# ZhengyiLuo/PULSE

Hardware: NVIDIA H100
Metric: env-steps/sec at 16384 humanoid envs, 1/2/4/8 H100; obs-kernel HBM GB/s (higher is better)
Workload: dtype bf16 GEMM operands, fp32 accumulate / master weights / observations

## Files before the change

### include/pulse_b200.h

```cpp
#ifndef PULSE_B200_H_
#define PULSE_B200_H_

#include <stdint.h>

#ifdef __cplusplus
extern "C" {
#endif

#define PULSE_ABI_VERSION 3

enum pulse_status {
  PULSE_OK = 0,
  PULSE_ERR_ARG = -1,
  PULSE_ERR_CUDA = -2,
  PULSE_ERR_UNSUPPORTED = -3
};

#define PULSE_NUM_BODIES 24
#define PULSE_NUM_DOF 69
#define PULSE_BODY_STATE_W 13
#define PULSE_SELF_OBS 358
#define PULSE_TASK_OBS_V6 576
#define PULSE_IM_OBS (PULSE_SELF_OBS + PULSE_TASK_OBS_V6)
#define PULSE_AMP_OBS 196
// ... 232 lines not shown

typedef struct {
  const float* bias;
  int32_t act;
  int32_t gate_mode;
  const pulse_bf16_t* gate;
  int64_t ldg;
  float alpha;
  pulse_bf16_t* out;
  int64_t ldo;
  pulse_bf16_t* out_t;
  int64_t ldot;
  float* out_f32;
  int64_t ldf;
  int64_t split_stride;
  pulse_bf16_t* preact;
  int64_t ldp;
  float* colsum;
  int32_t accumulate;
  int32_t reserved;
  double* sumsq;
  uint32_t* relu_mask; int64_t ld_rmask;
  const uint32_t* gate_mask; int64_t ld_gmask;
} pulse_gemm_epilogue_t;

#define PULSE_GEMM_A_MN 1u
#define PULSE_GEMM_B_MN 2u

int pulse_gemm_bf16(const void* a, int64_t lda, const void* b, int64_t ldb, int64_t m, int64_t n, int64_t k,
                    const pulse_gemm_epilogue_t* ep, int32_t split_k, uint32_t flags, void* stream);
int pulse_gemm_num_splits(int64_t k, int32_t split_k);
int pulse_gemm_tile_n(int64_t m, int64_t n, int64_t k, int32_t split_k, int32_t sms);
int pulse_gemm_last_tile_n(void);

int pulse_normalize_to_bf16(const float* x, int64_t ldx, int64_t rows, int64_t cols, const float* mean, const float* rstd,
                            pulse_bf16_t* out, int64_t ld_out, pulse_bf16_t* out_t, int64_t ld_t, float pad_one, void* stream);

int pulse_column_moments(const float* x, int64_t ldx, int64_t rows, int64_t cols, double* sums, void* stream);

int pulse_normalize_moments(const float* x, int64_t ldx, int64_t rows, int64_t cols, const float* mean, const float* rstd,
                            pulse_bf16_t* out, int64_t ld_out, double* sums, float pad_one, void* stream);

int pulse_normalize_split(const float* x, int64_t ldx, int64_t rows, int64_t cols, int64_t self_cols, const float* mean, const float* rstd,
                          pulse_bf16_t* p, int64_t ldp, int64_t p_off, pulse_bf16_t* t, int64_t ldt, double* sums, void* stream);

int pulse_rms_merge(double* sums, int64_t n, int32_t size, double* mean, double* var, double* count, float eps,
                    float* mean_f32, float* rstd_f32, void* stream);

int pulse_head1_forward(const pulse_bf16_t* h, int64_t ldh, int64_t rows, int32_t k, const pulse_bf16_t* w, const float* bias, float* out,
                        int64_t ldo, void* stream);

#define PULSE_HEAD1_MAX_CTAS 264
int pulse_head1_backward(const pulse_bf16_t* h, int64_t ldh, int64_t rows, int32_t k, const pulse_bf16_t* dv, int64_t ld_dv,
                         const pulse_bf16_t* w, pulse_bf16_t* dh, int64_t ld_dh, float* dw, float* db, float* dbias_prev, float* partials,
                         void* stream);

int pulse_ordered_sum_add(const float* x, int64_t n, int64_t stride_n, int64_t rows, int64_t cols, int64_t ld, float* out, int64_t ldo,
                          void* stream);

int pulse_gaussian_sample(const float* mu, int64_t ld_mu, const float* eps, const float* logstd, int64_t rows, int32_t num_actions,
                          float* actions, float* neglogp, void* stream);

typedef struct {
  const float* mu; int64_t ld_mu;
  const float* value; int64_t ld_value;
  const float* actions;
// ... 304 lines not shown
```

### pulse_b200/_lib.py

```python
import ctypes as C
import os

_PKG = os.path.dirname(os.path.abspath(__file__))
LIB_PATH = os.path.join(_PKG, "libpulse_b200.so")


class PulseError(RuntimeError):
    pass


c_float_p = C.POINTER(C.c_float)
c_i64_p = C.POINTER(C.c_int64)
c_i32_p = C.POINTER(C.c_int32)
c_u8_p = C.POINTER(C.c_uint8)
c_f64_p = C.POINTER(C.c_double)


class MotionLibDesc(C.Structure):
    _fields_ = [
        ("gts", C.c_void_p), ("grs", C.c_void_p), ("lrs", C.c_void_p), ("gvs", C.c_void_p), ("gavs", C.c_void_p),
        ("dvs", C.c_void_p), ("motion_aa", C.c_void_p), ("lengths", C.c_void_p), ("dt", C.c_void_p),
        ("num_frames", C.c_void_p), ("length_starts", C.c_void_p), ("total_frames", C.c_int64),
        ("num_motions", C.c_int64), ("frame_rec", C.c_void_p), ("aux_rec", C.c_void_p),
    ]
# ... 282 lines not shown
HEAD1_MAX_CTAS = 264
ACT_NONE, ACT_RELU, ACT_SILU = 0, 1, 2
Z_SAMPLE, Z_MEAN, Z_RESIDUAL = 0, 1, 2
STEP_REWARD, STEP_RESET, STEP_OBS, STEP_ALL, STEP_ADVANCE = 1, 2, 4, 7, 8
GETUP_REF, GETUP_FALL, GETUP_RECOVERY = 1, 2, 3

SIGNATURES = {
    "pulse_abi_version": (C.c_int, []),
    "pulse_last_error": (C.c_char_p, []),
    "pulse_launch_count": (C.c_int64, []),
    "pulse_motionlib_create": (C.c_int, [C.POINTER(MotionLibDesc), C.c_void_p, C.POINTER(C.c_void_p)]),
    "pulse_motionlib_destroy": (C.c_int, [C.c_void_p]),
    "pulse_motion_state": (C.c_int, [C.c_void_p, C.POINTER(MotionQuery), C.c_int64, C.c_void_p]),
    "pulse_im_step": (C.c_int, [C.c_void_p, C.POINTER(ImStepArgs), C.c_int64, C.c_void_p]),
    "pulse_reset_ref_state": (C.c_int, [C.c_void_p, C.POINTER(ResetArgs), C.c_int64, C.c_void_p]),
    "pulse_reset_getup": (C.c_int, [C.c_void_p, C.POINTER(GetupResetArgs), C.c_int64, C.c_void_p]),
    "pulse_getup_amp_init": (C.c_int, [C.POINTER(GetupAmpArgs), C.c_int64, C.c_void_p]),
    "pulse_policy_post": (C.c_int, [C.POINTER(PolicyPostArgs), C.c_int64, C.c_void_p]),
    "pulse_value_post": (C.c_int, [C.c_void_p, C.c_int64, C.c_void_p, C.c_void_p, C.c_float, C.c_void_p, C.c_void_p, C.c_int64, C.c_int64, C.c_void_p]),
    "pulse_amp_obs_row": (C.c_int, [C.POINTER(AmpRowArgs), C.c_int64, C.c_void_p]),
    "pulse_bump_counter": (C.c_int, [C.c_void_p, C.c_uint64, C.c_void_p]),
    "pulse_event_create": (C.c_int, [C.POINTER(C.c_void_p)]),
    "pulse_event_destroy": (C.c_int, [C.c_void_p]),
    "pulse_event_record": (C.c_int, [C.c_void_p, C.c_void_p]),
    "pulse_event_elapsed_ms": (C.c_int, [C.c_void_p, C.c_void_p, C.POINTER(C.c_float)]),
    "pulse_amp_obs": (C.c_int, [C.POINTER(AmpObsArgs), C.c_int64, C.c_void_p]),
    "pulse_gae": (C.c_int, [C.POINTER(GaeArgs), C.c_int32, C.c_int64, C.c_void_p]),
    "pulse_normalize_advantages": (C.c_int, [C.c_void_p, C.c_void_p, C.c_int64, C.c_void_p]),
    "pulse_gemm_bf16": (C.c_int, [C.c_void_p, C.c_int64, C.c_void_p, C.c_int64, C.c_int64, C.c_int64, C.c_int64,
                                  C.POINTER(GemmEpilogue), C.c_int32, C.c_uint32, C.c_void_p]),
    "pulse_gemm_num_splits": (C.c_int, [C.c_int64, C.c_int32]),
    "pulse_gemm_tile_n": (C.c_int, [C.c_int64, C.c_int64, C.c_int64, C.c_int32, C.c_int32]),
    "pulse_gemm_last_tile_n": (C.c_int, []),
    "pulse_normalize_to_bf16": (C.c_int, [C.c_void_p, C.c_int64, C.c_int64, C.c_int64, C.c_void_p, C.c_void_p, C.c_void_p, C.c_int64,
                                          C.c_void_p, C.c_int64, C.c_float, C.c_void_p]),
    "pulse_normalize_moments": (C.c_int, [C.c_void_p, C.c_int64, C.c_int64, C.c_int64, C.c_void_p, C.c_void_p, C.c_void_p, C.c_int64,
                                          C.c_void_p, C.c_float, C.c_void_p]),
    "pulse_normalize_split": (C.c_int, [C.c_void_p, C.c_int64, C.c_int64, C.c_int64, C.c_int64, C.c_void_p, C.c_void_p, C.c_void_p, C.c_int64,
                                        C.c_int64, C.c_void_p, C.c_int64, C.c_void_p, C.c_void_p]),
    "pulse_head1_forward": (C.c_int, [C.c_void_p, C.c_int64, C.c_int64, C.c_int32, C.c_void_p, C.c_void_p, C.c_void_p, C.c_int64, C.c_void_p]),
    "pulse_head1_backward": (C.c_int, [C.c_void_p, C.c_int64, C.c_int64, C.c_int32, C.c_void_p, C.c_int64, C.c_void_p, C.c_void_p, C.c_int64,
                                       C.c_void_p, C.c_void_p, C.c_void_p, C.c_void_p, C.c_void_p]),
    "pulse_ordered_sum_add": (C.c_int, [C.c_void_p, C.c_int64, C.c_int64, C.c_int64, C.c_int64, C.c_int64, C.c_void_p, C.c_int64, C.c_void_p]),
    "pulse_column_moments": (C.c_int, [C.c_void_p, C.c_int64, C.c_int64, C.c_int64, C.c_void_p, C.c_void_p]),
    "pulse_rms_merge": (C.c_int, [C.c_void_p, C.c_int64, C.c_int32, C.c_void_p, C.c_void_p, C.c_void_p, C.c_float, C.c_void_p, C.c_void_p,
                                  C.c_void_p]),
    "pulse_gaussian_sample": (C.c_int, [C.c_void_p, C.c_int64, C.c_void_p, C.c_void_p, C.c_int64, C.c_int32, C.c_void_p, C.c_void_p,
                                        C.c_void_p]),
    "pulse_ppo_loss": (C.c_int, [C.POINTER(PpoLossArgs), C.c_int64, C.c_void_p]),
    "pulse_disc_loss": (C.c_int, [C.c_void_p, C.c_int64, C.c_int64, C.c_int64, C.c_float, C.c_void_p, C.c_int64, C.c_void_p, C.c_void_p]),
    "pulse_relu_mask_scale": (C.c_int, [C.c_void_p, C.c_int64, C.c_int64, C.c_int64, C.c_void_p, C.c_void_p, C.c_int64, C.c_void_p]),
    "pulse_weight_reg": (C.c_int, [C.POINTER(WeightReg), C.c_void_p]),
    "pulse_axpy": (C.c_int, [C.c_float, C.c_void_p, C.c_void_p, C.c_int64, C.c_void_p]),
    "pulse_column_sum_bf16": (C.c_int, [C.c_void_p, C.c_int64, C.c_int64, C.c_int64, C.c_void_p, C.c_void_p]),
    "pulse_reduce_slabs": (C.c_int, [C.c_void_p, C.c_int64, C.c_int32, C.c_int64, C.c_void_p, C.c_void_p]),
    "pulse_sum_squares": (C.c_int, [C.c_void_p, C.c_int64, C.c_void_p, C.c_void_p]),
    "pulse_adam_step": (C.c_int, [C.c_void_p, C.c_void_p, C.c_void_p, C.c_void_p, C.c_int64, C.c_void_p, C.c_float, C.c_float,
                                  C.c_float, C.c_float, C.c_float, C.c_void_p, C.c_void_p, C.c_uint32, C.c_void_p, C.c_void_p]),
    "pulse_peer_reduce_adam": (C.c_int, [C.POINTER(PeerAdamArgs), C.c_void_p]),
    "pulse_refresh_weight_bf16": (C.c_int, [C.c_void_p, C.c_int64, C.c_int64, C.c_void_p, C.c_int64, C.c_void_p, C.c_int64, C.c_void_p]),
    "pulse_normalize_cols": (C.c_int, [C.c_void_p, C.c_int64, C.c_int64, C.c_int64, C.c_void_p, C.c_void_p, C.c_float, C.c_void_p, C.c_int64,
                                       C.c_int64, C.c_void_p]),
    "pulse_copy_cols_bf16": (C.c_int, [C.c_void_p, C.c_int64, C.c_int64, C.c_int64, C.c_void_p, C.c_int64, C.c_void_p, C.c_int64, C.c_void_p]),
    "pulse_vae_reparam": (C.c_int, [C.c_void_p, C.c_int64, C.c_void_p, C.c_int64, C.c_int64, C.c_int32, C.c_int32, C.c_int32, C.c_float,
                                    C.c_float, C.c_void_p, C.c_int64, C.c_void_p, C.c_int64, C.c_void_p]),
    "pulse_vae_reparam_philox": (C.c_int, [C.c_void_p, C.c_int64, C.c_int64, C.c_int32, C.c_int32, C.c_float, C.c_float, C.c_uint64,
# ... 84 lines not shown
```

### pulse_b200/csrc/gemm_kernel.inc

```

template <bool A_MN, bool B_MN, int MODE, int S, int BN>
__global__ void __launch_bounds__(kThreads, 1) gemm_bf16_kernel(const __grid_constant__ CUtensorMap map_a,
                                                                const __grid_constant__ CUtensorMap map_b,
                                                                const __grid_constant__ CUtensorMap map_c,
                                                                const __grid_constant__ CUtensorMap map_p,
                                                                const pulse_gemm_epilogue_t ep, int M, int N, int K,
                                                                int kb_per_split, int splits, int tma_out) {
  constexpr bool kFwd = MODE == kModeGeneric || MODE == kModeFwd;
  constexpr bool kDgrad = MODE == kModeGeneric || MODE == kModeDgrad || MODE == kModeDgradVec;
  constexpr bool kGateVec = MODE == kModeGeneric || MODE == kModeDgradVec;
  constexpr bool kAccum = MODE == kModeGeneric || MODE == kModeWgrad;
  constexpr bool kBf16Out = MODE != kModeWgrad;
  constexpr bool kRegEpi = MODE == kModeFwd || MODE == kModeDgrad;
  constexpr bool kWide = BN == kWideBN;
  constexpr bool kStaged = S == kStages && !kWide;
  static_assert(kStaged || kRegEpi, "deep-ring and wide instantiations run the register-resident epilogue only");
  static_assert(!kWide || (S == kStages && !A_MN), "wide tiles: 4-stage ring, K-major A");
  constexpr bool kPreRoom = sizeof(GemmSmem<S, BN>::epi[0]) >= 32768;
  extern __shared__ unsigned char gsm_raw[];
  GemmSmem<S, BN>& sm = *reinterpret_cast<GemmSmem<S, BN>*>((reinterpret_cast<uintptr_t>(gsm_raw) + 1023) & ~static_cast<uintptr_t>(1023));
  const int warp = threadIdx.x >> 5, lane = threadIdx.x & 31;
  const int work0 = static_cast<int>(blockIdx.x);
  const int work_stride = static_cast<int>(gridDim.x);
  const int tiles_n = (N + BN - 1) / BN, tiles_m = (M + BM - 1) / BM;
  const int tiles = tiles_m * tiles_n;
  const int total = tiles * splits;
  const int num_kb_total = (K + BK - 1) / BK;
  if (threadIdx.x == 0) PULSE_TRACE_START();

  if (threadIdx.x == 0) {
#pragma unroll
    for (int s = 0; s < S; ++s) {
      g_mbar_init(&sm.full[s], 1);
      g_mbar_init(&sm.empty[s], kConsumerWarps);
    }
    asm volatile("fence.mbarrier_init.release.cluster;\n" ::: "memory");
    asm volatile("prefetch.tensormap [%0];\n" ::"l"(&map_a) : "memory");
    asm volatile("prefetch.tensormap [%0];\n" ::"l"(&map_b) : "memory");
  }
  __syncthreads();
  if (threadIdx.x == 0) PULSE_TRACE(1);
  asm volatile("griddepcontrol.launch_dependents;\n" ::: "memory");

  if (warp < 4) {
    if constexpr (kWide) asm volatile("setmaxnreg.dec.sync.aligned.u32 %0;\n" ::"n"(kWideProducerRegs));
    if (warp == 0 && lane == 0) {
      asm volatile("griddepcontrol.wait;\n" ::: "memory");
      PULSE_TRACE(2);
      int it = 0, lw = 0;
      for (int w = work0; w < total; w += work_stride, ++lw) {
        const int split = w / tiles, t = w - split * tiles;
        const int m0 = (t / tiles_n) * BM, n0 = (t % tiles_n) * BN;
        const int kb0 = split * kb_per_split;
        const int num_kb = min(kb_per_split, num_kb_total - kb0);
        long long empty_clk = 0;
        (void)empty_clk;
        if (lw < 3) PULSE_TRACE_SET(25 + lw, num_kb);
        for (int kb = 0; kb < num_kb; ++kb, ++it) {
          const int s = it % S;
          PULSE_RING_WAIT(&sm.empty[s], ((it / S) & 1) ^ 1, empty_clk);
          g_mbar_expect_tx(&sm.full[s], kStageBytesA + BN * BK * 2);
          const int kk = (kb0 + kb) * BK;
          if (A_MN) {
            tma_load_2d(sm.a[s], &map_a, m0, kk, &sm.full[s]);
            tma_load_2d(sm.a[s] + 8192, &map_a, m0 + 64, kk, &sm.full[s]);
          } else {
            tma_load_2d(sm.a[s], &map_a, kk, m0, &sm.full[s]);
          }
          if (B_MN) {
#pragma unroll
            for (int i = 0; i < BN / 64; ++i) tma_load_2d(sm.b[s] + 8192 * i, &map_b, n0 + 64 * i, kk, &sm.full[s]);
          } else {
            tma_load_2d(sm.b[s], &map_b, kk, n0, &sm.full[s]);
          }
        }
        if (lw < 3) PULSE_TRACE_SET(28 + lw, empty_clk);
      }
    }
  } else {
    if constexpr (kWide) asm volatile("setmaxnreg.inc.sync.aligned.u32 %0;\n" ::"n"(kWideConsumerRegs));
    const int wg = (warp >> 2) - 1;
    const int ew = warp - 4;
    const int quarter = wg * 2 + (warp & 1);
    const int chalf = (warp >> 1) & 1;
    float* red_stage = nullptr;
    float* acc_s = nullptr;
    if constexpr (kStaged) {
      red_stage = sm.red[ew];
      acc_s = sm.epi[wg];
    }
    asm volatile("griddepcontrol.wait;\n" ::: "memory");
    int it = 0, lw = 0;
    for (int w = work0; w < total; w += work_stride, ++lw) {
      const int split = w / tiles, t = w - split * tiles;
      const int m0 = (t / tiles_n) * BM, n0 = (t % tiles_n) * BN;
      const int kb0 = split * kb_per_split;
      const int num_kb = min(kb_per_split, num_kb_total - kb0);
      const bool reg_epi = !kStaged || (kRegEpi && tma_out);
      const int r0 = (warp & 3) * 16 + (lane >> 2);
      const int row = m0 + quarter * 32 + lane;
      const bool row_ok = row < M;
      const bool gate_fast = kStaged && (MODE == kModeGeneric || MODE == kModeDgrad) && ep.gate != nullptr && ep.gate_mask == nullptr && ep.gate_mode == PULSE_ACT_RELU && (ep.ldg & 7) == 0 && n0 + chalf * kCols + kCols <= N;
      unsigned gmask[BN / 16] = {};
      const bool gate_bits = kDgrad && ep.gate_mask != nullptr;
      if (gate_bits && reg_epi) {
#pragma unroll
        for (int c = 0; c < BN / 32; ++c) {
#pragma unroll
          for (int h = 0; h < 2; ++h) {
            const int r = m0 + wg * 64 + r0 + 8 * h;
            if (r < M && n0 + c * 32 < N) gmask[2 * c + h] = __ldg(ep.gate_mask + static_cast<long long>((n0 >> 5) + c) * ep.ld_gmask + r);
          }
        }
      } else if (gate_bits && row_ok) {
#pragma unroll
        for (int cc = 0; cc < kChunks; ++cc) {
          const int col = n0 + (chalf * kChunks + cc) * 32;
          if (col < N) gmask[cc] = __ldg(ep.gate_mask + static_cast<long long>(col >> 5) * ep.ld_gmask + row);
        }
      }
      if (gate_fast && row_ok) {
        const uint4* g = reinterpret_cast<const uint4*>(reinterpret_cast<const __nv_bfloat16*>(ep.gate) + static_cast<long long>(row) * ep.ldg +
                                                        n0 + chalf * kCols);
        uint4 u[kChunks * 4];
#pragma unroll
        for (int i = 0; i < kChunks * 4; ++i) u[i] = __ldg(g + i);
#pragma unroll
        for (int i = 0; i < kChunks * 4; ++i) {
// ... 22 lines not shown
          const int t = (warp & 3) * 32 + lane;
          sm.bias[wg][t] = n0 + t < N ? __ldg(ep.bias + n0 + t) : 0.0f;
        }
      } else if (kFwd && ep.bias != nullptr) {
#pragma unroll
        for (int cc = 0; cc < kChunks; ++cc) {
          const int col = n0 + (chalf * kChunks + cc) * 32 + lane;
          if (col < N) bias_l[cc] = __ldg(ep.bias + col);
        }
      }

      float d[BN / 2];
#pragma unroll
      for (int i = 0; i < BN / 2; ++i) d[i] = 0.0f;
      acc_fence(d);
      int prev_s = -1;
      long long full_clk = 0;
      (void)full_clk;
      for (int kb = 0; kb < num_kb; ++kb, ++it) {
        const int s = it % S;
        PULSE_RING_WAIT(&sm.full[s], (it / S) & 1, full_clk);
        if (it == 0 && ew == 0 && lane == 0) PULSE_TRACE(3);
        wgmma_fence();
        const unsigned a_addr = s_u32(sm.a[s]) + static_cast<unsigned>(wg) * 8192u, b_addr = s_u32(sm.b[s]);
#pragma unroll
        for (int k = 0; k < BK / MMA_K; ++k) {
          const unsigned long long da = A_MN ? gmma_desc(a_addr + k * 2048, 8192) : gmma_desc(a_addr + k * 32, 16);
          const unsigned long long db = B_MN ? gmma_desc(b_addr + k * 2048, 8192) : gmma_desc(b_addr + k * 32, 16);
          if constexpr (kWide) wgmma_m64n256<A_MN ? 1 : 0, B_MN ? 1 : 0>(d, da, db, (kb | k) != 0 ? 1u : 0u);
          else wgmma_m64n128<A_MN ? 1 : 0, B_MN ? 1 : 0>(d, da, db, (kb | k) != 0 ? 1u : 0u);
        }
        wgmma_commit();
        wgmma_wait<1>();
        if (prev_s >= 0 && lane == 0) g_mbar_arrive(&sm.empty[prev_s]);
        prev_s = s;
      }
      wgmma_wait<0>();
      acc_fence(d);
      if (lane == 0) g_mbar_arrive(&sm.empty[prev_s]);
      if (ew == 0 && lane == 0 && lw < 3) {
        PULSE_TRACE(4 + lw);
        PULSE_TRACE_SET(22 + lw, full_clk);
      }

      if (kRegEpi && (warp & 3) == 0 && lane == 0) asm volatile("cp.async.bulk.wait_group.read 0;\n" ::: "memory");
      wg_sync(wg);
      float sq = 0.0f;

      if (reg_epi) {
        const int q = lane & 3;
        if (ep.alpha != 1.0f) {
#pragma unroll
          for (int i = 0; i < BN / 2; ++i) d[i] *= ep.alpha;
        }
        if (kFwd && ep.bias != nullptr) {
#pragma unroll
          for (int j = 0; j < BN / 8; ++j) {
            float2 b;
            if constexpr (kWide) {
              const int c = n0 + 8 * j + 2 * q;
              b = make_float2(c < N ? __ldg(ep.bias + c) : 0.0f, c + 1 < N ? __ldg(ep.bias + c + 1) : 0.0f);
            } else {
              b = *reinterpret_cast<const float2*>(sm.bias[wg] + 2 * q + 8 * j);
            }
            d[4 * j] += b.x; d[4 * j + 1] += b.y; d[4 * j + 2] += b.x; d[4 * j + 3] += b.y;
          }
        }
        if (kFwd && ep.relu_mask != nullptr) {
#pragma unroll
          for (int hf = 0; hf < BN / 128; ++hf) {
            unsigned wd[4][2];
#pragma unroll
// ... 275 lines not shown
              for (int i = 0; i < 32; ++i)
                if (col0 + i < N) p[i] = v[i];
            }
          }
          if (kBf16Out && ep.out != nullptr) {
            if (full && (ep.ldo & 7) == 0) {
              store_block_bf16(reinterpret_cast<uint4*>(red_stage), v,
                               reinterpret_cast<__nv_bfloat16*>(ep.out) + static_cast<long long>(m0 + quarter * 32) * ep.ldo + col0, ep.ldo,
                               M - (m0 + quarter * 32), lane);
            } else if (row_ok) {
              __nv_bfloat16* p = reinterpret_cast<__nv_bfloat16*>(ep.out) + static_cast<long long>(row) * ep.ldo + col0;
  #pragma unroll
              for (int i = 0; i < 32; ++i)
                if (col0 + i < N) p[i] = __float2bfloat16(v[i]);
            }
          }
          if (kFwd && ep.out_t != nullptr && row_ok) {
  #pragma unroll
            for (int i = 0; i < 32; ++i)
              if (col0 + i < N)
                reinterpret_cast<__nv_bfloat16*>(ep.out_t)[static_cast<long long>(col0 + i) * ep.ldot + row] = __float2bfloat16(v[i]);
          }
        }
        if (MODE == kModeWgrad && tma_out) {
          if (lane == 0) asm volatile("cp.async.bulk.wait_group.read 0;\n" ::: "memory");
          __syncwarp();
        }
        if (kDgrad && ep.sumsq != nullptr) add_sumsq(ep.sumsq, sq);
        if (ew == 0 && lane == 0 && lw < 3) PULSE_TRACE(17 + 2 * lw);
      }
    }
  }
  if ((MODE == kModeWgrad || kRegEpi) && warp >= 4 && lane == 0) asm volatile("cp.async.bulk.wait_group 0;\n" ::: "memory");
  if (threadIdx.x == 0) PULSE_TRACE(10);
}
```

### pulse_b200/csrc/gemm_wgmma.cu

```cuda
#include <cuda.h>
#include <stdlib.h>
#include <string.h>
#include <cuda_bf16.h>

#include "pulse_common.cuh"

namespace pulse {
namespace {

#ifndef PULSE_GEMM_VARIANT
#define PULSE_GEMM_VARIANT 0
#endif
constexpr int BM = 128, BK = 64, MMA_K = 16;
constexpr int kNarrowBN = 128, kWideBN = 256;
constexpr int kConsumerWarps = 8;
constexpr int kThreads = 128 + 32 * kConsumerWarps;
constexpr int kCols = 64;
constexpr int kChunks = kCols / 32;
constexpr int kStages = 4;
constexpr int kTmaOutF32 = 2;
constexpr unsigned kStageBytesA = BM * BK * 2;
constexpr int kWideProducerRegs = 40, kWideConsumerRegs = 232;

template <int S, int BN>
// ... 31 lines not shown
              "GEMM shared-memory layout exceeds the per-block opt-in limit");

__device__ __forceinline__ unsigned s_u32(const void* p) { return static_cast<unsigned>(__cvta_generic_to_shared(p)); }
__device__ __forceinline__ void g_mbar_init(unsigned long long* bar, unsigned count) {
  asm volatile("mbarrier.init.shared::cta.b64 [%0], %1;\n" ::"r"(s_u32(bar)), "r"(count));
}
__device__ __forceinline__ void g_mbar_expect_tx(unsigned long long* bar, unsigned bytes) {
  asm volatile("mbarrier.arrive.expect_tx.shared::cta.b64 _, [%0], %1;\n" ::"r"(s_u32(bar)), "r"(bytes) : "memory");
}
__device__ __forceinline__ void g_mbar_arrive(unsigned long long* bar) {
  asm volatile("mbarrier.arrive.shared::cta.b64 _, [%0];\n" ::"r"(s_u32(bar)) : "memory");
}
__device__ __forceinline__ bool g_mbar_try(unsigned long long* bar, unsigned parity) {
  unsigned ok;
  asm volatile(
      "{\n\t.reg .pred p;\n\t"
      "mbarrier.try_wait.parity.shared::cta.b64 p, [%1], %2;\n\t"
      "selp.u32 %0, 1, 0, p;\n\t}\n"
      : "=r"(ok)
      : "r"(s_u32(bar)), "r"(parity)
      : "memory");
  return ok != 0;
}
__device__ __forceinline__ void g_mbar_wait(unsigned long long* bar, unsigned parity) {
  for (int spin = 0; spin < (1 << 26); ++spin)
    if (g_mbar_try(bar, parity)) return;
  __trap();
}
__device__ __forceinline__ void tma_load_2d(void* smem_dst, const CUtensorMap* map, int c0, int c1, unsigned long long* bar) {
  asm volatile("cp.async.bulk.tensor.2d.shared::cluster.global.mbarrier::complete_tx::bytes [%0], [%1, {%3, %4}], [%2];\n" ::"r"(
                   s_u32(smem_dst)),
               "l"(map), "r"(s_u32(bar)), "r"(c0), "r"(c1)
               : "memory");
}
__device__ __forceinline__ void tma_store_2d(const CUtensorMap* map, unsigned smem_src, int c0, int c1) {
  asm volatile("cp.async.bulk.tensor.2d.global.shared::cta.bulk_group [%0, {%2, %3}], [%1];\n" ::"l"(map), "r"(smem_src), "r"(c0), "r"(c1)
               : "memory");
}
__device__ __forceinline__ void tma_store_3d(const CUtensorMap* map, unsigned smem_src, int c0, int c1, int c2) {
  asm volatile("cp.async.bulk.tensor.3d.global.shared::cta.bulk_group [%0, {%2, %3, %4}], [%1];\n" ::"l"(map), "r"(smem_src), "r"(c0), "r"(c1),
               "r"(c2)
               : "memory");
}
__device__ __forceinline__ void stmatrix_x4(unsigned addr, const unsigned (&r)[4]) {
  asm volatile("stmatrix.sync.aligned.m8n8.x4.shared.b16 [%0], {%1, %2, %3, %4};\n" ::"r"(addr), "r"(r[0]), "r"(r[1]), "r"(r[2]), "r"(r[3])
               : "memory");
}
__device__ __forceinline__ unsigned bf16x2_bits(__nv_bfloat162 h) { return *reinterpret_cast<unsigned*>(&h); }
__device__ __forceinline__ void add_sumsq(double* sumsq, float sq) {
#pragma unroll
  for (int o = 16; o > 0; o >>= 1) sq += __shfl_xor_sync(0xffffffffu, sq, o);
  if ((threadIdx.x & 31) == 0) atomicAdd(sumsq, static_cast<double>(sq));
}
__device__ __forceinline__ void wg_sync(int wg) { asm volatile("bar.sync %0, 128;\n" ::"r"(1 + wg) : "memory"); }

__device__ __forceinline__ unsigned long long gmma_desc(unsigned smem_addr, unsigned lbo) {
  unsigned long long d = 0;
  d |= static_cast<unsigned long long>((smem_addr >> 4) & 0x3fffu);
  d |= static_cast<unsigned long long>((lbo >> 4) & 0x3fffu) << 16;
  d |= static_cast<unsigned long long>(1024u >> 4) << 32;
  d |= static_cast<unsigned long long>(1u) << 62;
  return d;
}
__device__ __forceinline__ void wgmma_fence() { asm volatile("wgmma.fence.sync.aligned;\n" ::: "memory"); }
__device__ __forceinline__ void wgmma_commit() { asm volatile("wgmma.commit_group.sync.aligned;\n" ::: "memory"); }
template <int N>
// ... 137 lines not shown
  float2 f = __bfloat1622float2(z);
  f.x = __fdividef(f.x, 1.0f + __expf(-f.x));
  f.y = __fdividef(f.y, 1.0f + __expf(-f.y));
  return __floats2bfloat162_rn(f.x, f.y);
}

template <int ACT>
__device__ __forceinline__ void stage_tile_bf16(const float* d, unsigned stage, bool pre, int n0, int N) {
  const int lane = threadIdx.x & 31, warp = threadIdx.x >> 5;
  const unsigned srow = stage + ((warp & 3) * 16 + ((lane >> 3) & 1) * 8 + (lane & 7)) * 128;
  const int sj = lane >> 4;
  const __nv_bfloat162 zero2 = __float2bfloat162_rn(0.0f);
#pragma unroll
  for (int j = 0; j < kNarrowBN / 8; j += 2) {
    const bool full_half = n0 + 64 * (j >> 3) + 64 <= N;
    unsigned o[4], p[4];
#pragma unroll
    for (int k = 0; k < 4; ++k) {
      const int i = 4 * (j + (k >> 1)) + 2 * (k & 1);
      __nv_bfloat162 h = __floats2bfloat162_rn(d[i], d[i + 1]);
      p[k] = bf16x2_bits(h);
      if (ACT == PULSE_ACT_RELU) h = __hmax2(h, zero2);
      if (ACT == PULSE_ACT_SILU) h = full_half ? silu_bf16x2(h) : __floats2bfloat162_rn(act_apply(d[i], ACT), act_apply(d[i + 1], ACT));
      o[k] = bf16x2_bits(h);
    }
    const unsigned addr = srow + (j >> 3) * 8192 + ((((j & 7) + sj) ^ (lane & 7)) << 4);
    stmatrix_x4(addr, o);
    if (pre) stmatrix_x4(addr + 16384, p);
  }
}

enum : int { kModeGeneric = 0, kModeFwd = 1, kModeDgrad = 2, kModeWgrad = 3, kModeDgradVec = 4 };

#include "gemm_kernel.inc"

typedef CUresult (*EncodeTiledFn)(CUtensorMap*, CUtensorMapDataType, cuuint32_t, void*, const cuuint64_t*, const cuuint64_t*,
                                  const cuuint32_t*, const cuuint32_t*, CUtensorMapInterleave, CUtensorMapSwizzle,
                                  CUtensorMapL2promotion, CUtensorMapFloatOOBfill);
EncodeTiledFn get_encode_fn() {
  static EncodeTiledFn fn = nullptr;
  if (fn == nullptr) {
    void* p = nullptr;
    cudaDriverEntryPointQueryResult q;
    if (cudaGetDriverEntryPoint("cuTensorMapEncodeTiled", &p, cudaEnableDefault, &q) == cudaSuccess && q == cudaDriverEntryPointSuccess)
      fn = reinterpret_cast<EncodeTiledFn>(p);
  }
  return fn;
}

bool make_map(CUtensorMap* map, const void* base, long long rows, long long cols, long long ld, unsigned box_rows) {
  EncodeTiledFn fn = get_encode_fn();
  if (fn == nullptr) return false;
  cuuint64_t dims[2] = {static_cast<cuuint64_t>(cols), static_cast<cuuint64_t>(rows)};
  cuuint64_t strides[1] = {static_cast<cuuint64_t>(ld) * 2};
  cuuint32_t box[2] = {BK, box_rows};
  cuuint32_t estr[2] = {1, 1};
  return fn(map, CU_TENSOR_MAP_DATA_TYPE_BFLOAT16, 2, const_cast<void*>(base), dims, strides, box, estr, CU_TENSOR_MAP_INTERLEAVE_NONE,
            CU_TENSOR_MAP_SWIZZLE_128B, CU_TENSOR_MAP_L2_PROMOTION_L2_256B, CU_TENSOR_MAP_FLOAT_OOB_FILL_NONE) == CUDA_SUCCESS;
}

bool make_map_c(CUtensorMap* map, const float* base, long long rows, long long cols, long long ld) {
  EncodeTiledFn fn = get_encode_fn();
  if (fn == nullptr) return false;
  cuuint64_t dims[2] = {static_cast<cuuint64_t>(cols), static_cast<cuuint64_t>(rows)};
  cuuint64_t strides[1] = {static_cast<cuuint64_t>(ld) * 4};
  cuuint32_t box[2] = {32, 32};
// ... 67 lines not shown
  const char* e = getenv("PULSE_GEMM_STAGES");
  const bool force4 = e != nullptr && atoi(e) == kStages;
  return (!reg_epi || force4) ? kStages : preact ? 5 : 6;
}

constexpr int kWideMinKb = 4;
int gemm_tile_n(long long m, long long n, int kb_per_item, int splits, int sms) {
  if (n < kWideBN || kb_per_item < kWideMinKb || sms < 1) return kNarrowBN;
  const long long tm = (m + BM - 1) / BM;
  const long long rounds_narrow = (tm * ((n + kNarrowBN - 1) / kNarrowBN) * splits + sms - 1) / sms;
  const long long rounds_wide = (tm * ((n + kWideBN - 1) / kWideBN) * splits + sms - 1) / sms;
  return 2 * rounds_wide <= rounds_narrow ? kWideBN : kNarrowBN;
}

bool narrow_forced() {
  const char* e = getenv("PULSE_GEMM_BN");
  return e != nullptr && atoi(e) == kNarrowBN;
}
int g_last_tile_n = 0;

template <typename Kernel>
int set_smem_once(Kernel kernel, size_t bytes, bool* done) {
  if (*done) return PULSE_OK;
  int dev = 0, optin = 0;
  PULSE_CUDA_OK(cudaGetDevice(&dev));
  PULSE_CUDA_OK(cudaDeviceGetAttribute(&optin, cudaDevAttrMaxSharedMemoryPerBlockOptin, dev));
  PULSE_REQUIRE(bytes <= static_cast<size_t>(optin), "pulse_gemm_bf16: the GEMM needs %zu bytes of shared memory per block, the device allows %d",
                bytes, optin);
  PULSE_CUDA_OK(cudaFuncSetAttribute(kernel, cudaFuncAttributeMaxDynamicSharedMemorySize, static_cast<int>(bytes)));
  *done = true;
  return PULSE_OK;
}

template <bool A_MN, bool B_MN, int MODE, int S, int BN>
int launch_gemm_ring(const CUtensorMap& map_a, const CUtensorMap& map_b, const CUtensorMap& map_c, const CUtensorMap& map_p,
                     const pulse_gemm_epilogue_t& ep, int m, int n, int k, int splits, int kb_per_split, int tma_out, cudaStream_t stream) {
  static bool attr_set = false;
  const int rc = set_smem_once(gemm_bf16_kernel<A_MN, B_MN, MODE, S, BN>, smem_bytes<S, BN>(), &attr_set);
  if (rc != PULSE_OK) return rc;
  const int num_sms = gemm_num_sms();
  PULSE_REQUIRE(num_sms > 0, "pulse_gemm_bf16: cannot query the device's SM count");
  const long long total = static_cast<long long>((n + BN - 1) / BN) * ((m + BM - 1) / BM) * splits;
  const unsigned grid = static_cast<unsigned>(total < num_sms ? total : num_sms);
  static int use_pdl = -1;
  if (use_pdl < 0) {
    const char* e = getenv("PULSE_GEMM_PDL");
    use_pdl = (e != nullptr && e[0] == '0') ? 0 : 1;
  }
  cudaLaunchConfig_t cfg = {};
  cfg.gridDim = dim3(grid, 1, 1);
  cfg.blockDim = dim3(kThreads, 1, 1);
  cfg.dynamicSmemBytes = smem_bytes<S, BN>();
  cfg.stream = stream;
  cudaLaunchAttribute attr[1];
  int na = 0;
  if (use_pdl) {
    attr[na].id = cudaLaunchAttributeProgrammaticStreamSerialization;
    attr[na].val.programmaticStreamSerializationAllowed = 1;
    ++na;
  }
  cfg.attrs = attr;
  cfg.numAttrs = na;
  PULSE_CUDA_OK(cudaLaunchKernelEx(&cfg, gemm_bf16_kernel<A_MN, B_MN, MODE, S, BN>, map_a, map_b, map_c, map_p, ep, m, n, k, kb_per_split, splits, tma_out));
  PULSE_LAUNCH_OK("gemm_bf16_kernel");
  g_last_tile_n = BN;
  return PULSE_OK;
}

template <bool A_MN, bool B_MN, int MODE>
int launch_gemm(const CUtensorMap& map_a, const CUtensorMap& map_b, const void* b, long long ldb, const pulse_gemm_epilogue_t& ep, int m, int n,
                int k, int splits, int kb_per_split, cudaStream_t stream) {
  CUtensorMap map_c, map_p;
  int tma_out = 0;
  const int rc = epilogue_maps(MODE, ep, m, n, splits, &map_c, &map_p, &tma_out);
  if (rc != PULSE_OK) return rc;
  if constexpr (MODE == kModeFwd || MODE == kModeDgrad) {
    const int s = ring_stages(tma_out != 0, ep.preact != nullptr);
    if (s == kStages && tma_out == kTmaOutF32) tma_out = 0;
    if constexpr (!A_MN) {
      if (s != kStages && tma_out == 1 && ep.preact == nullptr && !narrow_forced() &&
          gemm_tile_n(m, n, kb_per_split, splits, gemm_num_sms()) == kWideBN) {
        CUtensorMap map_bw = map_b;
        if (!B_MN && !make_map(&map_bw, b, n, k, ldb, kWideBN)) {
          set_error("pulse_gemm_bf16: cuTensorMapEncodeTiled failed for the wide B operand");
          return PULSE_ERR_CUDA;
        }
        return launch_gemm_ring<A_MN, B_MN, MODE, kStages, kWideBN>(map_a, map_bw, map_c, map_p, ep, m, n, k, splits, kb_per_split, tma_out, stream);
      }
    }
    if (s == 6) return launch_gemm_ring<A_MN, B_MN, MODE, 6, kNarrowBN>(map_a, map_b, map_c, map_p, ep, m, n, k, splits, kb_per_split, tma_out, stream);
    if constexpr (MODE == kModeFwd) {
      if (s == 5) return launch_gemm_ring<A_MN, B_MN, MODE, 5, kNarrowBN>(map_a, map_b, map_c, map_p, ep, m, n, k, splits, kb_per_split, tma_out, stream);
    }
  }
  return launch_gemm_ring<A_MN, B_MN, MODE, kStages, kNarrowBN>(map_a, map_b, map_c, map_p, ep, m, n, k, splits, kb_per_split, tma_out, stream);
}

int epilogue_mode(const pulse_gemm_epilogue_t* ep) {
  const bool want_fwd = ep->bias || ep->act != PULSE_ACT_NONE || ep->preact || ep->out_t || ep->relu_mask;
  const bool want_dgrad = ep->gate || ep->colsum || ep->sumsq || ep->gate_mask;
  const bool want_accum = ep->accumulate != 0;
  if (!want_dgrad && !want_accum) return kModeFwd;
  if (!want_fwd && !want_accum) return (ep->gate && ep->gate_mode != PULSE_ACT_RELU) ? kModeDgradVec : kModeDgrad;
  if (!want_fwd && !want_dgrad && !ep->out) return kModeWgrad;
  return kModeGeneric;
}

}
}

#if PULSE_GEMM_VARIANT == 3
extern "C" int pulse_debug_gemm_trace(long long* out) {
  return cudaMemcpyFromSymbol(out, pulse::g_gemm_trace, sizeof(long long) * 32) == cudaSuccess ? 0 : -2;
}
#endif

extern "C" int pulse_gemm_num_splits(int64_t k, int32_t split_k) {
  const int num_kb = static_cast<int>((k + 63) / 64);
  int splits = split_k < 1 ? 1 : (split_k > num_kb ? num_kb : split_k);
  const int kb_per_split = (num_kb + splits - 1) / splits;
  return (num_kb + kb_per_split - 1) / kb_per_split;
}

extern "C" int pulse_gemm_tile_n(int64_t m, int64_t n, int64_t k, int32_t split_k, int32_t sms) {
  const int num_kb = static_cast<int>((k + 63) / 64);
  const int splits = pulse_gemm_num_splits(k, split_k);
  return pulse::gemm_tile_n(m, n, (num_kb + splits - 1) / splits, splits, sms);
}

extern "C" int pulse_gemm_last_tile_n(void) { return pulse::g_last_tile_n; }

extern "C" int pulse_gemm_bf16(const void* a, int64_t lda, const void* b, int64_t ldb, int64_t m, int64_t n, int64_t k,
                               const pulse_gemm_epilogue_t* ep, int32_t split_k, uint32_t flags, void* stream) {
  using namespace pulse;
  PULSE_REQUIRE(a && b && ep, "pulse_gemm_bf16: null argument");
  PULSE_REQUIRE(m > 0 && n > 0 && k > 0, "pulse_gemm_bf16: empty problem %lld x %lld x %lld", (long long)m, (long long)n, (long long)k);
  PULSE_REQUIRE(m < (1ll << 31) && n < (1ll << 31) && k < (1ll << 31), "pulse_gemm_bf16: dimension too large");
  PULSE_REQUIRE((flags & ~3u) == 0, "pulse_gemm_bf16: bad flags");
  const bool a_mn = flags & PULSE_GEMM_A_MN, b_mn = flags & PULSE_GEMM_B_MN;
  PULSE_REQUIRE(lda >= (a_mn ? m : k) && ldb >= (b_mn ? n : k) && (lda % 8) == 0 && (ldb % 8) == 0,
                "pulse_gemm_bf16: leading dimensions must cover the contiguous extent and be multiples of 8 (16-byte rows), got %lld %lld",
                (long long)lda, (long long)ldb);
  PULSE_REQUIRE(aligned16(a) && aligned16(b), "pulse_gemm_bf16: operands must be 16-byte aligned");
  PULSE_REQUIRE(ep->out || ep->out_t || ep->out_f32, "pulse_gemm_bf16: no output requested");
  PULSE_REQUIRE(split_k >= 1, "pulse_gemm_bf16: split_k must be >= 1");
  PULSE_REQUIRE(split_k == 1 || (ep->out_f32 && !ep->out && !ep->out_t && !ep->bias && ep->act == PULSE_ACT_NONE && !ep->gate && !ep->preact && !ep->colsum),
                "pulse_gemm_bf16: split-K only supports plain fp32 outputs (slabs or atomic accumulation)");
  PULSE_REQUIRE(ep->gate == nullptr || ep->gate_mode == PULSE_ACT_RELU || ep->gate_mode == PULSE_ACT_SILU, "pulse_gemm_bf16: bad gate_mode");
  PULSE_REQUIRE((ep->relu_mask == nullptr || ep->ld_rmask >= m) && (ep->gate_mask == nullptr || ep->ld_gmask >= m),
                "pulse_gemm_bf16: mask word rows must hold at least M entries");
  PULSE_REQUIRE(!(ep->gate_mask && ep->gate), "pulse_gemm_bf16: give the ReLU gate either as bf16 activations or as bit words, not both");
  CUtensorMap map_a, map_b;
  const bool ok_a = a_mn ? make_map(&map_a, a, k, m, lda, 64) : make_map(&map_a, a, m, k, lda, BM);
  const bool ok_b = b_mn ? make_map(&map_b, b, k, n, ldb, 64) : make_map(&map_b, b, n, k, ldb, kNarrowBN);
  if (!ok_a || !ok_b) {
    set_error("pulse_gemm_bf16: cuTensorMapEncodeTiled failed (driver entry point missing or bad strides)");
    return PULSE_ERR_CUDA;
  }
  const int num_kb = static_cast<int>((k + BK - 1) / BK);
  const int splits = pulse_gemm_num_splits(k, split_k);
  const int kb_per_split = (num_kb + splits - 1) / splits;
  cudaStream_t st = static_cast<cudaStream_t>(stream);
  const int mode = epilogue_mode(ep);
// ... 16 lines not shown
```

Measured before the change: 2.047 million.

## Pair GEMM CTAs into clusters that multicast shared B tiles via TMA

Adds a 2-CTA cluster path for MN-major A and B GEMMs (wgrad and fp32-output forward). Each CTA in a pair works on an adjacent M-tile with the same N-tile. Each CTA loads one 64-column half of the B box and multicasts it to both CTAs, which halves B traffic from L2/HBM. Empty barriers now count consumers across the cluster, so slots are released remotely. The cost is cluster synchronisation, tighter coupling between paired CTAs, and fewer schedulable slots.

```diff
diff --git a/include/pulse_b200.h b/include/pulse_b200.h
--- a/include/pulse_b200.h
+++ b/include/pulse_b200.h
@@ -288,6 +288,8 @@
 int pulse_gemm_num_splits(int64_t k, int32_t split_k);
 int pulse_gemm_tile_n(int64_t m, int64_t n, int64_t k, int32_t split_k, int32_t sms);
 int pulse_gemm_last_tile_n(void);
+int pulse_gemm_last_cluster(void);
+int pulse_gemm_schedule(int64_t m, int64_t n, int64_t k, int32_t split_k, int32_t grid, int32_t cluster, int32_t* out, int64_t cap);
 
 int pulse_normalize_to_bf16(const float* x, int64_t ldx, int64_t rows, int64_t cols, const float* mean, const float* rstd,
                             pulse_bf16_t* out, int64_t ld_out, pulse_bf16_t* out_t, int64_t ld_t, float pad_one, void* stream);
diff --git a/pulse_b200/_lib.py b/pulse_b200/_lib.py
--- a/pulse_b200/_lib.py
+++ b/pulse_b200/_lib.py
@@ -338,6 +338,8 @@
     "pulse_gemm_num_splits": (C.c_int, [C.c_int64, C.c_int32]),
     "pulse_gemm_tile_n": (C.c_int, [C.c_int64, C.c_int64, C.c_int64, C.c_int32, C.c_int32]),
     "pulse_gemm_last_tile_n": (C.c_int, []),
+    "pulse_gemm_last_cluster": (C.c_int, []),
+    "pulse_gemm_schedule": (C.c_int, [C.c_int64, C.c_int64, C.c_int64, C.c_int32, C.c_int32, C.c_int32, C.c_void_p, C.c_int64]),
     "pulse_normalize_to_bf16": (C.c_int, [C.c_void_p, C.c_int64, C.c_int64, C.c_int64, C.c_void_p, C.c_void_p, C.c_void_p, C.c_int64,
                                           C.c_void_p, C.c_int64, C.c_float, C.c_void_p]),
     "pulse_normalize_moments": (C.c_int, [C.c_void_p, C.c_int64, C.c_int64, C.c_int64, C.c_void_p, C.c_void_p, C.c_void_p, C.c_int64,
diff --git a/pulse_b200/csrc/gemm_kernel.inc b/pulse_b200/csrc/gemm_kernel.inc
--- a/pulse_b200/csrc/gemm_kernel.inc
+++ b/pulse_b200/csrc/gemm_kernel.inc
@@ -1,5 +1,5 @@
 
-template <bool A_MN, bool B_MN, int MODE, int S, int BN>
+template <bool A_MN, bool B_MN, int MODE, int S, int BN, int CL>
 __global__ void __launch_bounds__(kThreads, 1) gemm_bf16_kernel(const __grid_constant__ CUtensorMap map_a,
                                                                 const __grid_constant__ CUtensorMap map_b,
                                                                 const __grid_constant__ CUtensorMap map_c,
@@ -16,15 +16,16 @@
   constexpr bool kStaged = S == kStages && !kWide;
   static_assert(kStaged || kRegEpi, "deep-ring and wide instantiations run the register-resident epilogue only");
   static_assert(!kWide || (S == kStages && !A_MN), "wide tiles: 4-stage ring, K-major A");
+  static_assert(CL == 1 || (CL == 2 && B_MN && BN == 128), "clusters: pairs of CTAs sharing the two 64-column B boxes of a narrow tile");
   constexpr bool kPreRoom = sizeof(GemmSmem<S, BN>::epi[0]) >= 32768;
   extern __shared__ unsigned char gsm_raw[];
   GemmSmem<S, BN>& sm = *reinterpret_cast<GemmSmem<S, BN>*>((reinterpret_cast<uintptr_t>(gsm_raw) + 1023) & ~static_cast<uintptr_t>(1023));
   const int warp = threadIdx.x >> 5, lane = threadIdx.x & 31;
-  const int work0 = static_cast<int>(blockIdx.x);
-  const int work_stride = static_cast<int>(gridDim.x);
+  const int rank = CL > 1 ? static_cast<int>(cluster_ctarank()) : 0;
+  const int work0 = static_cast<int>(blockIdx.x) / CL;
+  const int work_stride = static_cast<int>(gridDim.x) / CL;
   const int tiles_n = (N + BN - 1) / BN, tiles_m = (M + BM - 1) / BM;
-  const int tiles = tiles_m * tiles_n;
-  const int total = tiles * splits;
+  const int total = tiles_m / CL * tiles_n * splits;
   const int num_kb_total = (K + BK - 1) / BK;
   if (threadIdx.x == 0) PULSE_TRACE_START();
 
@@ -32,13 +33,14 @@
 #pragma unroll
     for (int s = 0; s < S; ++s) {
       g_mbar_init(&sm.full[s], 1);
-      g_mbar_init(&sm.empty[s], kConsumerWarps);
+      g_mbar_init(&sm.empty[s], kConsumerWarps * CL);
     }
     asm volatile("fence.mbarrier_init.release.cluster;\n" ::: "memory");
     asm volatile("prefetch.tensormap [%0];\n" ::"l"(&map_a) : "memory");
     asm volatile("prefetch.tensormap [%0];\n" ::"l"(&map_b) : "memory");
   }
-  __syncthreads();
+  if constexpr (CL > 1) cluster_sync();
+  else __syncthreads();
   if (threadIdx.x == 0) PULSE_TRACE(1);
   asm volatile("griddepcontrol.launch_dependents;\n" ::: "memory");
 
@@ -49,8 +51,8 @@
       PULSE_TRACE(2);
       int it = 0, lw = 0;
       for (int w = work0; w < total; w += work_stride, ++lw) {
-        const int split = w / tiles, t = w - split * tiles;
-        const int m0 = (t / tiles_n) * BM, n0 = (t % tiles_n) * BN;
+        const GemmItem item = gemm_item(w, rank, tiles_m, tiles_n, CL);
+        const int split = item.split, m0 = item.mt * BM, n0 = item.nt * BN;
         const int kb0 = split * kb_per_split;
         const int num_kb = min(kb_per_split, num_kb_total - kb0);
         long long empty_clk = 0;
@@ -67,7 +69,9 @@
           } else {
             tma_load_2d(sm.a[s], &map_a, kk, m0, &sm.full[s]);
           }
-          if (B_MN) {
+          if constexpr (CL > 1) {
+            tma_load_2d_mc(sm.b[s] + 8192 * rank, &map_b, n0 + 64 * rank, kk, &sm.full[s], static_cast<unsigned short>((1u << CL) - 1u));
+          } else if (B_MN) {
 #pragma unroll
             for (int i = 0; i < BN / 64; ++i) tma_load_2d(sm.b[s] + 8192 * i, &map_b, n0 + 64 * i, kk, &sm.full[s]);
           } else {
@@ -91,9 +95,14 @@
     }
     asm volatile("griddepcontrol.wait;\n" ::: "memory");
     int it = 0, lw = 0;
+    auto release = [&](int s) {
+      g_mbar_arrive(&sm.empty[s]);
+#pragma unroll
+      for (int r = 1; r < CL; ++r) g_mbar_arrive_cluster(&sm.empty[s], static_cast<unsigned>((rank + r) % CL));
+    };
     for (int w = work0; w < total; w += work_stride, ++lw) {
-      const int split = w / tiles, t = w - split * tiles;
-      const int m0 = (t / tiles_n) * BM, n0 = (t % tiles_n) * BN;
+      const GemmItem item = gemm_item(w, rank, tiles_m, tiles_n, CL);
+      const int split = item.split, m0 = item.mt * BM, n0 = item.nt * BN;
       const int kb0 = split * kb_per_split;
       const int num_kb = min(kb_per_split, num_kb_total - kb0);
       const bool reg_epi = !kStaged || (kRegEpi && tma_out);
@@ -182,12 +191,12 @@
         }
         wgmma_commit();
         wgmma_wait<1>();
-        if (prev_s >= 0 && lane == 0) g_mbar_arrive(&sm.empty[prev_s]);
+        if (prev_s >= 0 && lane == 0) release(prev_s);
         prev_s = s;
       }
       wgmma_wait<0>();
       acc_fence(d);
-      if (lane == 0) g_mbar_arrive(&sm.empty[prev_s]);
+      if (lane == 0) release(prev_s);
       if (ew == 0 && lane == 0 && lw < 3) {
         PULSE_TRACE(4 + lw);
         PULSE_TRACE_SET(22 + lw, full_clk);
@@ -529,5 +538,6 @@
     }
   }
   if ((MODE == kModeWgrad || kRegEpi) && warp >= 4 && lane == 0) asm volatile("cp.async.bulk.wait_group 0;\n" ::: "memory");
+  if constexpr (CL > 1) cluster_sync();
   if (threadIdx.x == 0) PULSE_TRACE(10);
 }
diff --git a/pulse_b200/csrc/gemm_wgmma.cu b/pulse_b200/csrc/gemm_wgmma.cu
--- a/pulse_b200/csrc/gemm_wgmma.cu
+++ b/pulse_b200/csrc/gemm_wgmma.cu
@@ -87,6 +87,30 @@
                    s_u32(smem_dst)),
                "l"(map), "r"(s_u32(bar)), "r"(c0), "r"(c1)
                : "memory");
+}
+__device__ __forceinline__ void tma_load_2d_mc(void* smem_dst, const CUtensorMap* map, int c0, int c1, unsigned long long* bar,
+                                               unsigned short cta_mask) {
+  asm volatile(
+      "cp.async.bulk.tensor.2d.shared::cluster.global.mbarrier::complete_tx::bytes.multicast::cluster [%0], [%1, {%3, %4}], [%2], %5;\n" ::"r"(
+          s_u32(smem_dst)),
+      "l"(map), "r"(s_u32(bar)), "r"(c0), "r"(c1), "h"(cta_mask)
+      : "memory");
+}
+__device__ __forceinline__ void g_mbar_arrive_cluster(unsigned long long* bar, unsigned rank) {
+  asm volatile(
+      "{\n\t.reg .b32 ra;\n\t"
+      "mapa.shared::cluster.u32 ra, %0, %1;\n\t"
+      "mbarrier.arrive.shared::cluster.b64 _, [ra];\n\t}\n" ::"r"(s_u32(bar)),
+      "r"(rank)
+      : "memory");
+}
+__device__ __forceinline__ unsigned cluster_ctarank() {
+  unsigned r;
+  asm volatile("mov.u32 %0, %%cluster_ctarank;\n" : "=r"(r));
+  return r;
+}
+__device__ __forceinline__ void cluster_sync() {
+  asm volatile("barrier.cluster.arrive.relaxed;\n\tbarrier.cluster.wait;\n" ::: "memory");
 }
 __device__ __forceinline__ void tma_store_2d(const CUtensorMap* map, unsigned smem_src, int c0, int c1) {
   asm volatile("cp.async.bulk.tensor.2d.global.shared::cta.bulk_group [%0, {%2, %3}], [%1];\n" ::"l"(map), "r"(smem_src), "r"(c0), "r"(c1)
@@ -290,6 +314,19 @@
 
 enum : int { kModeGeneric = 0, kModeFwd = 1, kModeDgrad = 2, kModeWgrad = 3, kModeDgradVec = 4 };
 
+struct GemmItem {
+  int split, mt, nt;
+};
+__host__ __device__ __forceinline__ GemmItem gemm_item(int w, int rank, int tiles_m, int tiles_n, int cl) {
+  const int groups = tiles_m / cl * tiles_n;
+  GemmItem it;
+  it.split = w / groups;
+  const int t = w - it.split * groups;
+  it.mt = (t / tiles_n) * cl + rank;
+  it.nt = t % tiles_n;
+  return it;
+}
+
 #include "gemm_kernel.inc"
 
 typedef CUresult (*EncodeTiledFn)(CUtensorMap*, CUtensorMapDataType, cuuint32_t, void*, const cuuint64_t*, const cuuint64_t*,
@@ -423,38 +460,63 @@
   return PULSE_OK;
 }
 
-template <bool A_MN, bool B_MN, int MODE, int S, int BN>
+bool cluster_disabled() {
+  const char* e = getenv("PULSE_GEMM_CLUSTER");
+  return e != nullptr && atoi(e) == 0;
+}
+int g_last_cluster = 0;
+
+template <bool A_MN, bool B_MN, int MODE, int S, int BN, int CL = 1>
 int launch_gemm_ring(const CUtensorMap& map_a, const CUtensorMap& map_b, const CUtensorMap& map_c, const CUtensorMap& map_p,
                      const pulse_gemm_epilogue_t& ep, int m, int n, int k, int splits, int kb_per_split, int tma_out, cudaStream_t stream) {
+  auto kernel = gemm_bf16_kernel<A_MN, B_MN, MODE, S, BN, CL>;
   static bool attr_set = false;
-  const int rc = set_smem_once(gemm_bf16_kernel<A_MN, B_MN, MODE, S, BN>, smem_bytes<S, BN>(), &attr_set);
+  const int rc = set_smem_once(kernel, smem_bytes<S, BN>(), &attr_set);
   if (rc != PULSE_OK) return rc;
   const int num_sms = gemm_num_sms();
   PULSE_REQUIRE(num_sms > 0, "pulse_gemm_bf16: cannot query the device's SM count");
-  const long long total = static_cast<long long>((n + BN - 1) / BN) * ((m + BM - 1) / BM) * splits;
-  const unsigned grid = static_cast<unsigned>(total < num_sms ? total : num_sms);
   static int use_pdl = -1;
   if (use_pdl < 0) {
     const char* e = getenv("PULSE_GEMM_PDL");
     use_pdl = (e != nullptr && e[0] == '0') ? 0 : 1;
   }
   cudaLaunchConfig_t cfg = {};
-  cfg.gridDim = dim3(grid, 1, 1);
   cfg.blockDim = dim3(kThreads, 1, 1);
   cfg.dynamicSmemBytes = smem_bytes<S, BN>();
   cfg.stream = stream;
-  cudaLaunchAttribute attr[1];
+  cudaLaunchAttribute attr[2];
   int na = 0;
   if (use_pdl) {
     attr[na].id = cudaLaunchAttributeProgrammaticStreamSerialization;
     attr[na].val.programmaticStreamSerializationAllowed = 1;
     ++na;
   }
+  const long long total = static_cast<long long>((n + BN - 1) / BN) * ((m + BM - 1) / BM) * splits / CL;
+  long long slots = num_sms / CL;
+  if constexpr (CL > 1) {
+    attr[na].id = cudaLaunchAttributeClusterDimension;
+    attr[na].val.clusterDim.x = CL;
+    attr[na].val.clusterDim.y = 1;
+    attr[na].val.clusterDim.z = 1;
+    ++na;
+    static int max_clusters = 0;
+    if (max_clusters == 0) {
+      cfg.gridDim = dim3(static_cast<unsigned>(slots * CL), 1, 1);
+      cfg.attrs = attr + na - 1;
+      cfg.numAttrs = 1;
+      PULSE_CUDA_OK(cudaOccupancyMaxActiveClusters(&max_clusters, kernel, &cfg));
+      PULSE_REQUIRE(max_clusters > 0, "pulse_gemm_bf16: no cluster of %d GEMM CTAs fits on the device", CL);
+    }
+    if (slots > max_clusters) slots = max_clusters;
+  }
+  const unsigned grid = static_cast<unsigned>((total < slots ? total : slots) * CL);
+  cfg.gridDim = dim3(grid, 1, 1);
   cfg.attrs = attr;
   cfg.numAttrs = na;
-  PULSE_CUDA_OK(cudaLaunchKernelEx(&cfg, gemm_bf16_kernel<A_MN, B_MN, MODE, S, BN>, map_a, map_b, map_c, map_p, ep, m, n, k, kb_per_split, splits, tma_out));
+  PULSE_CUDA_OK(cudaLaunchKernelEx(&cfg, kernel, map_a, map_b, map_c, map_p, ep, m, n, k, kb_per_split, splits, tma_out));
   PULSE_LAUNCH_OK("gemm_bf16_kernel");
   g_last_tile_n = BN;
+  g_last_cluster = CL;
   return PULSE_OK;
 }
 
@@ -465,9 +527,18 @@
   int tma_out = 0;
   const int rc = epilogue_maps(MODE, ep, m, n, splits, &map_c, &map_p, &tma_out);
   if (rc != PULSE_OK) return rc;
+  const bool pair = A_MN && B_MN && !cluster_disabled() && ((m + BM - 1) / BM) % 2 == 0 && gemm_num_sms() >= 2;
+  if constexpr (A_MN && B_MN && MODE == kModeWgrad) {
+    if (pair && tma_out == 1)
+      return launch_gemm_ring<A_MN, B_MN, MODE, kStages, kNarrowBN, 2>(map_a, map_b, map_c, map_p, ep, m, n, k, splits, kb_per_split, tma_out, stream);
+  }
   if constexpr (MODE == kModeFwd || MODE == kModeDgrad) {
     const int s = ring_stages(tma_out != 0, ep.preact != nullptr);
     if (s == kStages && tma_out == kTmaOutF32) tma_out = 0;
+    if constexpr (A_MN && B_MN && MODE == kModeFwd) {
+      if (pair && s == 6 && tma_out == kTmaOutF32)
+        return launch_gemm_ring<A_MN, B_MN, MODE, 6, kNarrowBN, 2>(map_a, map_b, map_c, map_p, ep, m, n, k, splits, kb_per_split, tma_out, stream);
+    }
     if constexpr (!A_MN) {
       if (s != kStages && tma_out == 1 && ep.preact == nullptr && !narrow_forced() &&
           gemm_tile_n(m, n, kb_per_split, splits, gemm_num_sms()) == kWideBN) {
@@ -520,6 +591,28 @@
 }
 
 extern "C" int pulse_gemm_last_tile_n(void) { return pulse::g_last_tile_n; }
+
+extern "C" int pulse_gemm_last_cluster(void) { return pulse::g_last_cluster; }
+
+extern "C" int pulse_gemm_schedule(int64_t m, int64_t n, int64_t k, int32_t split_k, int32_t grid, int32_t cluster, int32_t* out, int64_t cap) {
+  using namespace pulse;
+  PULSE_REQUIRE(m > 0 && n > 0 && k > 0 && m < (1ll << 31) && n < (1ll << 31) && k < (1ll << 31) && split_k >= 1, "pulse_gemm_schedule: bad shape");
+  PULSE_REQUIRE(out != nullptr && (cluster == 1 || cluster == 2) && grid >= cluster && grid % cluster == 0, "pulse_gemm_schedule: bad grid / cluster");
+  const int tiles_m = static_cast<int>((m + BM - 1) / BM), tiles_n = static_cast<int>((n + kNarrowBN - 1) / kNarrowBN);
+  PULSE_REQUIRE(tiles_m % cluster == 0, "pulse_gemm_schedule: %d m-tiles do not pair", tiles_m);
+  const int total = tiles_m / cluster * tiles_n * pulse_gemm_num_splits(k, split_k);
+  long long count = 0;
+  for (int cta = 0; cta < grid; ++cta) {
+    for (int w = cta / cluster; w < total; w += grid / cluster, ++count) {
+      PULSE_REQUIRE(count < cap, "pulse_gemm_schedule: more than %lld items", (long long)cap);
+      const GemmItem it = gemm_item(w, cta % cluster, tiles_m, tiles_n, cluster);
+      out[3 * count] = it.split;
+      out[3 * count + 1] = it.mt;
+      out[3 * count + 2] = it.nt;
+    }
+  }
+  return static_cast<int>(count);
+}
 
 extern "C" int pulse_gemm_bf16(const void* a, int64_t lda, const void* b, int64_t ldb, int64_t m, int64_t n, int64_t k,
                                const pulse_gemm_epilogue_t* ep, int32_t split_k, uint32_t flags, void* stream) {
```

After: 2.084 million (median of 6 runs). 1.02x the previous value.
